# skywoodsz/qm_control

Measured on AMD Instinct MI355X. Metric: MPC+WBC control steps/sec (24-DoF quadruped-manipulator, SQP horizon N=100), higher is better.
Workload: dtype f64; 1 GPU; C3/C4: trot gait, horizon N=100 (dt 0.015), 1024 random initial states per GPU (seed 1235), cold start, 1 SQP iteration + policy eval + 3-level WBC; back-to-back steps, the WBC of a step on its own stream beside the next step's MPC kernels (pipelined THROUGHPUT: the per-kernel times add up to more than ms_per_step; the unpipelined step latency is latency_ms); instances_per_gpu=1024, global_batch=1024, parallelism=shard1, all_status_ok=True, ls_trials=1, engine=hip, max_nodes=128

## Files before the change

### qm_control_amd/csrc/host/qm_pipeline.h

```cpp
#pragma once
#include <cstddef>
#include <cstdint>
#include <vector>
#include "../kernels/k_grid.h"
#include "../kernels/k_lq.h"
#include "../kernels/k_riccati.h"
#include "../kernels/k_ls.h"
#include "../kernels/k_ilqr.h"
#include "../kernels/k_ipm.h"

struct QmMpcBuffers {
  int Bmax = 0, nmax = 0, nref = 0, nev = 0;
  double* mb = nullptr; double* st = nullptr;
  double* t0 = nullptr; double* x0 = nullptr; double* ref_t = nullptr; double* ref_x = nullptr; double* ev = nullptr; int* modes = nullptr;
  int* n_nodes = nullptr; double* node_t = nullptr; double* node_ts = nullptr; double* node_dt = nullptr; int* node_ev = nullptr; int* node_mode = nullptr;
  double* zvel = nullptr; double* zpos = nullptr; double* xref = nullptr; double* eeref = nullptr; int* status = nullptr;
  double* x = nullptr; double* u = nullptr; double* dx = nullptr; double* du = nullptr; double* stage = nullptr; double* lqdbg = nullptr; double* kin = nullptr;
  double* perf = nullptr; double* base_sum = nullptr; double* perf_sum = nullptr; double* step_info = nullptr;
  double* alpha = nullptr; int* done = nullptr; double* xs = nullptr; double* us = nullptr; double* out_perf = nullptr;
  double* xt = nullptr; double* ut = nullptr;
  double* ipm_s = nullptr; double* ipm_l = nullptr; double* ipm_ds = nullptr; double* ipm_dl = nullptr; double* ipm_ratio = nullptr; double* ipm_info = nullptr;
  int* prev_n = nullptr; double* prev_t = nullptr; int* prev_ev = nullptr;
  int* open_cnt = nullptr; int* tickets = nullptr; int* host_open_dev = nullptr; volatile int* host_open = nullptr;
  int* ncap_dev = nullptr; int* host_ncap_dev = nullptr; volatile int* host_ncap = nullptr;
};

__host__ __device__ inline int qm_mpc_status(int k0_status, const double* step_info4, bool strict) {
  if (k0_status != 0) return k0_status;
  const double* s4 = step_info4; const int pv = (s4[3] == s4[3]) ? (int)s4[3] : 2;
  const bool finite = (s4[0] - s4[0] == 0.0) && (s4[1] - s4[1] == 0.0) && (s4[2] - s4[2] == 0.0);
  if (!finite || (pv & 2)) return -4;
  if (pv & 1) return strict ? -4 : QM_MPC_WARN_PIVOT;
  return 0;
}

template <class BK>
struct QmMpcPipeline {
  BK& bk; QmMpcBuffers d;
  int ls_trials_run = 0;
  bool ls_trials_pending = false; int ls_trials_cap = 0;
  double* p0_x = nullptr; double* p0_u = nullptr; int* p0_mode = nullptr; bool p0_enable = false; bool p0_done = false;
  bool defer_apply = false; int pending_apply_B = 0; int pending_apply_threads = 0;
  bool device_tail = true;
  int riccati_skip = 0;
  int lq_prof = 0;
  int solver = 0;
  bool r_blocks = false;
  bool r_force_dense = false;
  bool rblk() const { return r_blocks && !r_force_dense; }
  bool speculative_apply = true;
  bool ipm_fresh = true;
  int solved_B = 0;
  int ncap = 0;
  bool ncap_pending = false;
  bool has_m18 = true;
  const int* front_status = nullptr; int front_B = 0;
  explicit QmMpcPipeline(BK& b) : bk(b) {}

  template <class T> T* A(size_t n) { T* p = (T*)bk.alloc(n * sizeof(T)); bk.zero(p, n * sizeof(T)); return p; }

  void allocate(const double* mb_host, const double* st_host, int Bmax, int nmax, int nref, int nev, bool debug_lq) {
    d.Bmax = Bmax; d.nmax = nmax; d.nref = nref; d.nev = nev;
    const size_t NB = (size_t)nmax * Bmax;
    d.mb = A<double>(MB_SIZE); d.st = A<double>(ST_SIZE);
    bk.to_device(d.mb, mb_host, MB_SIZE * 8); bk.to_device(d.st, st_host, ST_SIZE * 8); note_settings(st_host);
    d.t0 = A<double>(Bmax); d.x0 = A<double>((size_t)Bmax * 30); d.ref_t = A<double>((size_t)Bmax * nref); d.ref_x = A<double>((size_t)Bmax * nref * QM_NREF);
    d.ev = A<double>((size_t)Bmax * nev); d.modes = A<int>((size_t)Bmax * (nev + 1));
    d.n_nodes = A<int>(Bmax); d.node_t = A<double>(NB); d.node_ts = A<double>(NB); d.node_dt = A<double>(NB); d.node_ev = A<int>(NB); d.node_mode = A<int>(NB);
    d.zvel = A<double>(NB * 4); d.zpos = A<double>(NB * 4); d.xref = A<double>(NB * 30); d.eeref = A<double>(NB * 7); d.status = A<int>(Bmax);
    d.x = A<double>(NB * 30); d.u = A<double>(NB * 30); d.dx = A<double>(NB * 30); d.du = A<double>(NB * 30);
    d.stage = A<double>(NB * SR_SIZE); d.lqdbg = debug_lq ? A<double>(NB * LQ_DBG_SIZE) : nullptr; d.kin = A<double>((NB + 64) * KR_SIZE);
    d.perf = A<double>(NB * PF_SIZE); d.base_sum = A<double>((size_t)Bmax * 4); d.perf_sum = A<double>((size_t)Bmax * 4); d.step_info = A<double>((size_t)Bmax * 4);
    d.alpha = A<double>(Bmax); d.done = A<int>(Bmax); d.xs = A<double>(NB * 30); d.us = A<double>(NB * 30); d.out_perf = A<double>((size_t)Bmax * 10);
    d.prev_n = A<int>(Bmax); d.prev_t = A<double>(NB); d.prev_ev = A<int>(NB);
    d.open_cnt = A<int>(QM_LS_MAX_TRIALS); d.tickets = A<int>(QM_LS_MAX_TRIALS);
    d.ncap_dev = A<int>(3); { void* hv = nullptr; d.host_ncap_dev = (int*)bk.alloc_mapped(sizeof(int), &hv); d.host_ncap = (volatile int*)hv; d.host_ncap[0] = 0; }
    { void* hv = nullptr; d.host_open_dev = (int*)bk.alloc_mapped(QM_LS_MAX_TRIALS * sizeof(int), &hv); d.host_open = (volatile int*)hv; for (int i = 0; i < QM_LS_MAX_TRIALS; ++i) d.host_open[i] = 0; }
  }
  void note_settings(const double* st_host) { r_blocks = qm_r_is_block_diagonal(st_host); }
  void release() {
    void* ps[] = {d.mb, d.st, d.t0, d.x0, d.ref_t, d.ref_x, d.ev, d.modes, d.n_nodes, d.node_t, d.node_ts, d.node_dt, d.node_ev, d.node_mode, d.zvel, d.zpos, d.xref, d.eeref, d.status,
                  d.x, d.u, d.dx, d.du, d.xt, d.ut, d.ipm_s, d.ipm_l, d.ipm_ds, d.ipm_dl, d.ipm_ratio, d.ipm_info, d.stage, d.lqdbg, d.kin, d.perf, d.base_sum, d.perf_sum, d.step_info, d.alpha, d.done, d.xs, d.us, d.out_perf, d.prev_n, d.prev_t, d.prev_ev, d.open_cnt, d.tickets, d.ncap_dev};
    for (void* p : ps) if (p) bk.free(p);
    if (d.host_open) bk.free_mapped((void*)d.host_open);
    if (d.host_ncap) bk.free_mapped((void*)d.host_ncap);
    d = QmMpcBuffers();
  }

  int ls_trials() {
    if (ls_trials_pending) { int oc[QM_LS_MAX_TRIALS]; bk.to_host(oc, d.open_cnt, sizeof(oc)); int t = 0; while (t < QM_LS_MAX_TRIALS && oc[t] > 0) ++t; ls_trials_run = (1 + t > ls_trials_cap) ? ls_trials_cap : 1 + t; ls_trials_pending = false; }
    return ls_trials_run;
  }

  void apply_pending() { if (!pending_apply_B) return; QmLsArgs l = ls_args(pending_apply_B); bk.launch(qm_ls_apply_kernel, (pending_apply_threads * 30 + 255) / 256, 256, 0, l); pending_apply_B = 0; }

  void upload_inputs(int B, const double* t0, const double* x0, const double* ref_t, const double* ref_x, const double* ev, const int* modes) {
    bk.to_device(d.t0, t0, (size_t)B * 8); bk.to_device(d.x0, x0, (size_t)B * 30 * 8);
    bk.to_device(d.ref_t, ref_t, (size_t)B * d.nref * 8); bk.to_device(d.ref_x, ref_x, (size_t)B * d.nref * QM_NREF * 8);
    bk.to_device(d.ev, ev, (size_t)B * d.nev * 8); bk.to_device(d.modes, modes, (size_t)B * (d.nev + 1) * 4);
  }

  QmLsArgs ls_args(int B) {
    QmLsArgs a; a.mb = d.mb; a.st = d.st; a.B = B; a.nmax = d.nmax; a.n_nodes = d.n_nodes; a.node_ts = d.node_ts; a.node_dt = d.node_dt; a.node_ev = d.node_ev; a.node_mode = d.node_mode;
    a.zvel = d.zvel; a.zpos = d.zpos; a.xref = d.xref; a.eeref = d.eeref; a.x0 = d.x0; a.x = d.x; a.u = d.u; a.dx = d.dx; a.du = d.du; a.alpha = d.alpha; a.done = d.done;
    a.perf = d.perf; a.perf_sum = d.perf_sum; a.base_sum = d.base_sum; a.step_info = d.step_info; a.xs = d.xs; a.us = d.us; a.out_perf = d.out_perf; a.trial = 0; a.max_trials = 0; a.node_t = d.node_t; a.p0_t = d.t0; a.p0_ev = d.ev; a.p0_modes = d.modes; a.p0_nev = d.nev; a.p0_x = nullptr; a.p0_u = nullptr; a.p0_mode = nullptr; a.with_alpha = 0; a.open_cnt = d.open_cnt; a.tickets = d.tickets; a.host_open = (volatile int*)d.host_open_dev; a.xt = nullptr; a.ut = nullptr; a.ilqr = 0; a.ipm_s = nullptr; a.ipm_ds = nullptr; a.ipm_info = nullptr;
    return a;
  }

  void grid(int B, double horizon, bool warm = false) {
    warm = warm && solved_B == B;
    if (warm) { QmSaveGridArgs sg; sg.B = B; sg.nmax = d.nmax; sg.n_nodes = d.n_nodes; sg.node_t = d.node_t; sg.node_ev = d.node_ev; sg.prev_n = d.prev_n; sg.prev_t = d.prev_t; sg.prev_ev = d.prev_ev;
                bk.launch(qm_save_grid_kernel, (d.nmax * B + 63) / 64, 64, 0, sg); }
    QmGridArgs g; g.mb = d.mb; g.st = d.st; g.B = B; g.nmax = d.nmax; g.nref = d.nref; g.nev = d.nev; g.t0 = d.t0; g.x0 = d.x0; g.ref_t = d.ref_t; g.ref_x = d.ref_x; g.ev = d.ev; g.modes = d.modes;
    g.horizon = horizon; g.n_nodes = d.n_nodes; g.node_t = d.node_t; g.node_ts = d.node_ts; g.node_dt = d.node_dt; g.node_ev = d.node_ev; g.node_mode = d.node_mode;
    g.zvel = d.zvel; g.zpos = d.zpos; g.xref = d.xref; g.eeref = d.eeref; g.x = d.x; g.u = d.u; g.status = d.status; g.front_status = (front_status && front_B == B) ? front_status : nullptr;
    if (ncap_pending) bk.wait_flag(d.host_ncap, -1);
    g.ncap_dev = d.ncap_dev; g.host_ncap = (volatile int*)d.host_ncap_dev; d.host_ncap[0] = -1; ncap = 0; ncap_pending = true;
    g.warm = warm ? 1 : 0; g.prev_n = d.prev_n; g.prev_t = d.prev_t; g.prev_ev = d.prev_ev; g.prev_xs = d.xs; g.prev_us = d.us;
    bk.launch(qm_grid_kernel, (B + 63) / 64, 64, 0, g);
    bk.launch(qm_grid_nodes_kernel, (d.nmax * B + 63) / 64, 64, 0, g);
    ipm_fresh = true;
  }
  void advance(int B, double dt) {
    QmAdvanceArgs v; v.B = B; v.nmax = d.nmax; v.n_nodes = d.n_nodes; v.node_t = d.node_t; v.node_ev = d.node_ev; v.xs = d.xs; v.dt = dt; v.t0 = d.t0; v.x0 = d.x0;
    bk.launch(qm_advance_kernel, (B + 63) / 64, 64, 0, v);
  }
  void sqp_iteration(int B, int max_trials = 14, bool last = false) {
    const bool ilqr = solver == 1, ipm = solver == 3;
    QmIpmArgs ia;
    if (ipm) {
      const size_t NBm = (size_t)d.nmax * d.Bmax;
      if (!d.ipm_s) { d.ipm_s = A<double>(NBm * QM_NH); d.ipm_l = A<double>(NBm * QM_NH); d.ipm_ds = A<double>(NBm * QM_NH); d.ipm_dl = A<double>(NBm * QM_NH); d.ipm_ratio = A<double>(NBm * 2); d.ipm_info = A<double>((size_t)d.Bmax * IPM_INFO); }
      ia.mb = d.mb; ia.st = d.st; ia.B = B; ia.nmax = d.nmax; ia.n_nodes = d.n_nodes; ia.node_ev = d.node_ev; ia.node_mode = d.node_mode; ia.node_dt = d.node_dt; ia.x = d.x; ia.u = d.u; ia.dx = d.dx; ia.du = d.du;
      ia.s = d.ipm_s; ia.lam = d.ipm_l; ia.ds = d.ipm_ds; ia.dlam = d.ipm_dl; ia.ratio = d.ipm_ratio; ia.info = d.ipm_info; ia.alpha = d.alpha; ia.done = d.done; ia.out_perf = d.out_perf;
      if (ipm_fresh) bk.launch(qm_ipm_init_kernel, (d.nmax * B + 63) / 64, 64, 0, ia);
      ipm_fresh = false;
    }
    if (ilqr && !d.xt) { d.xt = A<double>((size_t)d.nmax * d.Bmax * 30); d.ut = A<double>((size_t)d.nmax * d.Bmax * 30); }
    QmRolloutArgs ro; ro.mb = d.mb; ro.st = d.st; ro.B = B; ro.nmax = d.nmax; ro.mode = 0; ro.trial = 0; ro.n_nodes = d.n_nodes; ro.node_dt = d.node_dt; ro.node_ev = d.node_ev; ro.x0 = d.x0;
    ro.x = d.x; ro.u = d.u; ro.stage = d.stage; ro.alpha = d.alpha; ro.done = d.done; ro.xt = d.xt; ro.ut = d.ut;
    if (ilqr) bk.launch(qm_ilqr_rollout_kernel, B, 64, 0, ro);
    if (ncap == 0) { if (ncap_pending) bk.wait_flag(d.host_ncap, -1); const int word = ncap_pending ? d.host_ncap[0] : (d.nmax | (1 << 16)); ncap_pending = false;
                     ncap = word & 0xFFFF; has_m18 = (word >> 16) != 0; if (ncap < 1 || ncap > d.nmax) { ncap = d.nmax; has_m18 = true; } }
    const int nodes_threads = ncap * B;
    if (max_trials > QM_LS_MAX_TRIALS) max_trials = QM_LS_MAX_TRIALS;
    QmLqArgs q; q.mb = d.mb; q.st = d.st; q.B = B; q.nmax = d.nmax; q.n_nodes = d.n_nodes; q.node_ts = d.node_ts; q.node_dt = d.node_dt; q.node_ev = d.node_ev; q.node_mode = d.node_mode;
    q.zvel = d.zvel; q.zpos = d.zpos; q.xref = d.xref; q.eeref = d.eeref; q.x = d.x; q.u = d.u; q.stage = d.stage; q.perf = d.perf; q.dbg = d.lqdbg; q.kin = d.kin; q.prof = lq_prof; q.ncap = ncap;
    q.ipm_s = d.ipm_s; q.ipm_l = d.ipm_l; q.ipm_info = d.ipm_info; q.rb = rblk() ? 1 : 0; q.single_mt = has_m18 ? 0 : 1;
    q.i0 = 0;
    bk.launch(qm_lq_kin_kernel, (nodes_threads + 63) / 64, 64, LQ_KIN_LDS_BYTES, q);
    if (ipm) bk.launch(qm_lq_ipm_kernel, B * ncap, LW_BLOCK, LQ_LDS_BYTES, q);
    else if (d.lqdbg || lq_prof) bk.launch(qm_lq_dbg_kernel, B * ncap, LW_BLOCK, LQ_LDS_BYTES, q);
    else { bk.launch(qm_lq_kernel, B * ncap, LW_BLOCK, LQ_LDS_BYTES, q);
           if (has_m18) bk.launch(qm_lq_m18_kernel, B * ncap, LW_BLOCK, LQ_LDS_BYTES, q); }
    QmLsArgs l = ls_args(B); if (ilqr) { l.xt = d.xt; l.ut = d.ut; l.ilqr = 1; }
    if (ipm) { l.ipm_s = d.ipm_s; l.ipm_ds = d.ipm_ds; l.ipm_info = d.ipm_info; }
    QmRiccatiArgs r; r.B = B; r.nmax = d.nmax; r.n_nodes = d.n_nodes; r.node_ev = d.node_ev; r.x0 = d.x0; r.x = d.x; r.stage = d.stage; r.dx = d.dx; r.du = d.du; r.step_info = d.step_info; r.skip = riccati_skip;
    r.perf = d.perf; r.base_sum = d.base_sum; r.alpha = d.alpha; r.done = d.done; r.out_perf = d.out_perf; r.open_cnt = d.open_cnt; r.tickets = d.tickets;
    if (riccati_skip) bk.launch(qm_riccati_prof_kernel, B, RW_BLOCK, RW_LDS_BYTES, r);
    else bk.launch(qm_riccati_kernel, B, RW_BLOCK, RW_LDS_BYTES, r);
    if (ipm) { bk.launch(qm_ipm_dir_kernel, (d.nmax * B + 63) / 64, 64, 0, ia); bk.launch(qm_ipm_alpha_kernel, B, 64, 0, ia); }
    ls_trials_run = 0; ls_trials_pending = false; p0_done = false;
    if (device_tail && !ilqr && !ipm && max_trials >= 1) {
      l.trial = 0; l.max_trials = max_trials;
      if (p0_enable && last && p0_x) { l.p0_x = p0_x; l.p0_u = p0_u; l.p0_mode = p0_mode; p0_done = true; bk.wbc_inputs_next(); }
      if (rblk()) bk.launch(qm_ls_eval_kernel, (nodes_threads + 63) / 64, 64, LS_EVAL_LDS_BYTES, l); else bk.launch(qm_ls_eval_dense_kernel, (nodes_threads + 63) / 64, 64, LS_EVAL_LDS_BYTES, l);
      { QmLsArgs ls = l; ls.with_alpha = 1; ls.tickets = nullptr; bk.launch(qm_perf_sum_kernel, B, 64, 0, ls); }
      if (max_trials > 1) { QmLsArgs lt = l; lt.trial = 1;
        if (rblk()) bk.launch(qm_ls_tail_kernel, B, LS_TAIL_BLOCK, LS_TAIL_LDS_BYTES(d.nmax), lt); else bk.launch(qm_ls_tail_dense_kernel, B, LS_TAIL_BLOCK, LS_TAIL_LDS_BYTES(d.nmax), lt); }
      ls_trials_pending = true; ls_trials_cap = max_trials;
      if (defer_apply && last) { pending_apply_B = B; pending_apply_threads = nodes_threads; solved_B = B; return; }
      bk.launch(qm_ls_apply_kernel, (nodes_threads * 30 + 255) / 256, 256, 0, l);
      if (!last) bk.launch(qm_ls_commit_kernel, (nodes_threads * 30 + 255) / 256, 256, 0, l);
// ... 23 lines not shown
```

### qm_control_amd/csrc/host/qmhip.hip

```cpp
#include <hip/hip_runtime.h>
#include <chrono>
#include <cmath>
#include <cstdio>
#include <cstring>
#include <map>
#include <mutex>
#include <string>
#include <vector>
#include "../../../include/qmhip.h"
#include "qm_model_io.h"
#define QM_LQ_KERNELS_EXTERN 1
#include "qm_pipeline.h"
#include "qm_wbc_pipeline.h"
#include "qm_sim_pipeline.h"
#include "qm_front_pipeline.h"
#include "qm_hoqp_pipeline.h"
#include "qm_io_pipeline.h"
#include "qm_tick_pipeline.h"
#include "qm_publish_pipeline.h"

static thread_local std::string g_create_error;

#define QM_GUARD(c) std::unique_lock<std::recursive_mutex> qm_lk_; if (c) qm_lk_ = std::unique_lock<std::recursive_mutex>(const_cast<qmhip_ctx*>(c)->mu)
#define QM_NEED_MPC(c) do { if ((c) && (c)->wbc_only) { const_cast<qmhip_ctx*>(c)->fail(std::string(__func__) + ": not available on a WBC-only context (qmhip_create_wbc_context)"); return QMHIP_ERR_STATE; } } while (0)
#define HIP_TRY(ctx, expr) do { hipError_t e_ = (expr); if (e_ != hipSuccess) { (ctx)->fail(std::string(#expr) + ": " + hipGetErrorString(e_)); return QMHIP_ERR_HIP; } } while (0)

struct HipBackend {
  hipStream_t stream = nullptr;
  hipStream_t stream_b = nullptr;
  hipStream_t stream_c = nullptr;
  hipStream_t cur = nullptr;
  hipEvent_t ev_in = nullptr, ev_wbc = nullptr; bool wbc_pending = false;
  int profiling = 0;
  std::string error;
  struct Span { std::string name; hipEvent_t a, b; };
  std::vector<Span> spans; std::vector<hipEvent_t> pool;
  std::map<std::string, std::pair<double, int>> acc;
  std::map<const void*, int> lds_set;
  std::map<std::string, int> lds_pad;
  hipEvent_t ev() { if (!pool.empty()) { hipEvent_t e = pool.back(); pool.pop_back(); return e; } hipEvent_t e = nullptr; check(hipEventCreate(&e), "hipEventCreate"); return e; }
  void check(hipError_t e, const char* what) { if (e != hipSuccess && error.empty()) error = std::string(what) + ": " + hipGetErrorString(e); }
  template <class K> const char* name_of(K k) {
    const void* p = (const void*)k;
    if (p == (const void*)qm_grid_kernel || p == (const void*)qm_grid_nodes_kernel || p == (const void*)qm_save_grid_kernel || p == (const void*)qm_advance_kernel) return "grid"; if (p == (const void*)qm_lq_kernel || p == (const void*)qm_lq_dbg_kernel || p == (const void*)qm_lq_ipm_kernel) return "lq"; if (p == (const void*)qm_lq_m18_kernel) return "lq_m18"; if (p == (const void*)qm_lq_kin_kernel) return "lq_kin"; if (p == (const void*)qm_riccati_kernel || p == (const void*)qm_riccati_prof_kernel) return "riccati";
    if (p == (const void*)qm_ls_eval_kernel || p == (const void*)qm_ls_eval_dense_kernel || p == (const void*)qm_ls_eval_ipm_kernel) return "ls_eval";
    if (p == (const void*)qm_ipm_init_kernel || p == (const void*)qm_ipm_dir_kernel || p == (const void*)qm_ipm_alpha_kernel || p == (const void*)qm_ipm_commit_kernel || p == (const void*)qm_ipm_barrier_kernel) return "ipm"; if (p == (const void*)qm_ilqr_rollout_kernel) return "rollout"; if (p == (const void*)qm_sim_kernel) return "sim"; if (p == (const void*)qm_wbc_kernel || p == (const void*)qm_wbc_prof_kernel) return "wbc"; if (p == (const void*)qm_policy_kernel || p == (const void*)qm_policy_measured_kernel) return "policy"; if (p == (const void*)qm_policy_fb_kernel || p == (const void*)qm_policy_fb_pub_kernel) return "policy_fb"; if (p == (const void*)qm_policy_publish_kernel) return "publish"; if (p == (const void*)qm_hoqp_kernel) return "hoqp"; if (p == (const void*)qm_step_pack_kernel) return "io"; if (p == (const void*)qm_tick_state_kernel || p == (const void*)qm_tick_pack_kernel) return "tick";
    return "ls_misc";
  }
  template <class K, class A> void launch(K kernel, int grid, int block, size_t lds, const A& args) {
    if (grid <= 0) return;
    if (!lds_pad.empty()) { auto it = lds_pad.find(name_of(kernel)); if (it != lds_pad.end()) lds += (size_t)it->second; }
    if (lds > 48 * 1024) {
      const void* p = (const void*)kernel; auto it = lds_set.find(p);
      if (it == lds_set.end() || it->second < (int)lds) { check(hipFuncSetAttribute(p, hipFuncAttributeMaxDynamicSharedMemorySize, (int)lds), "hipFuncSetAttribute"); lds_set[p] = (int)lds; }
    }
    const void* kp_ = (const void*)kernel;
    const bool is_lq_ = kp_ == (const void*)qm_lq_kernel || kp_ == (const void*)qm_lq_m18_kernel || kp_ == (const void*)qm_lq_ipm_kernel;
    const bool span = profiling == 1 || (profiling == 3 && is_lq_) || (profiling == 2 && (kp_ == (const void*)qm_lq_kernel || kp_ == (const void*)qm_lq_m18_kernel || kp_ == (const void*)qm_lq_ipm_kernel || kp_ == (const void*)qm_riccati_kernel || kp_ == (const void*)qm_wbc_kernel));
    Span s; if (span) { s.name = name_of(kernel); s.a = ev(); s.b = ev(); check(hipEventRecord(s.a, cur), "hipEventRecord"); }
    hipLaunchKernelGGL(kernel, dim3(grid), dim3(block), lds, cur, args);
    check(hipGetLastError(), "kernel launch");
    if (span) { check(hipEventRecord(s.b, cur), "hipEventRecord"); spans.push_back(s); }
  }
  void resolve() {
    if (spans.empty()) return;
    hipStreamSynchronize(stream); hipStreamSynchronize(stream_b);
    for (auto& s : spans) { float ms = 0; hipEventElapsedTime(&ms, s.a, s.b); auto& a = acc[s.name]; a.first += ms; a.second += 1; pool.push_back(s.a); pool.push_back(s.b); }
    spans.clear();
  }
  void* alloc(size_t n) { void* p = nullptr; check(hipMalloc(&p, n ? n : 8), "hipMalloc"); return p; }
  void free(void* p) { hipFree(p); }
  void zero(void* p, size_t n) { check(hipMemsetAsync(p, 0, n, cur), "hipMemsetAsync"); }
  void to_device(void* d, const void* s, size_t n) { sync(); check(hipMemcpyAsync(d, s, n, hipMemcpyHostToDevice, stream), "H2D"); check(hipStreamSynchronize(stream), "sync"); }
  void to_host(void* d, const void* s, size_t n) { sync(); check(hipMemcpyAsync(d, s, n, hipMemcpyDeviceToHost, stream), "D2H"); check(hipStreamSynchronize(stream), "sync"); }
  void sync() { check(hipStreamSynchronize(stream), "sync"); check(hipStreamSynchronize(stream_b), "sync"); wbc_pending = false; }
  hipEvent_t ev_order = nullptr;
  void stream_select(int s) { cur = s ? stream_b : stream; }
  void stream_order(int a, int b) { if (!ev_order) check(hipEventCreateWithFlags(&ev_order, hipEventDisableTiming), "hipEventCreate"); check(hipEventRecord(ev_order, a ? stream_b : stream), "hipEventRecord"); check(hipStreamWaitEvent(b ? stream_b : stream, ev_order, 0), "hipStreamWaitEvent"); }
  void copy_dd(void* d, const void* s, size_t n) { check(hipMemcpyAsync(d, s, n, hipMemcpyDeviceToDevice, cur), "D2D"); }
  void* alloc_mapped(size_t n, void** host_view) { void* h = nullptr; void* dv = nullptr; check(hipHostMalloc(&h, n ? n : 8, hipHostMallocMapped), "hipHostMalloc"); check(hipHostGetDevicePointer(&dv, h, 0), "hipHostGetDevicePointer"); *host_view = h; return dv; }
  void free_mapped(void* host_view) { hipHostFree(host_view); }
  hipEvent_t ev_io_a = nullptr, ev_io_b = nullptr;
  void* alloc_pinned(size_t n) { void* h = nullptr; check(hipHostMalloc(&h, n ? n : 8, hipHostMallocDefault), "hipHostMalloc"); return h; }
  void free_pinned(void* p) { hipHostFree(p); }
  void* io_event() { hipEvent_t e = nullptr; check(hipEventCreateWithFlags(&e, hipEventDisableTiming), "hipEventCreate"); return (void*)e; }
  void io_event_free(void* e) { hipEventDestroy((hipEvent_t)e); }
  void copy_in(void* d, const void* s, size_t n, int on) { check(hipMemcpyAsync(d, s, n, hipMemcpyHostToDevice, on ? stream_b : stream), "H2D"); }
  void copy_out(void* d, const void* s, size_t n, void* done, bool wbc) {
    if (!ev_io_a) { check(hipEventCreateWithFlags(&ev_io_a, hipEventDisableTiming), "hipEventCreate"); check(hipEventCreateWithFlags(&ev_io_b, hipEventDisableTiming), "hipEventCreate"); }
    check(hipEventRecord(ev_io_a, stream), "hipEventRecord"); check(hipStreamWaitEvent(stream_c, ev_io_a, 0), "hipStreamWaitEvent");
    if (wbc) { check(hipEventRecord(ev_io_b, stream_b), "hipEventRecord"); check(hipStreamWaitEvent(stream_c, ev_io_b, 0), "hipStreamWaitEvent"); }
    check(hipMemcpyAsync(d, s, n, hipMemcpyDeviceToHost, stream_c), "D2H"); check(hipEventRecord((hipEvent_t)done, stream_c), "hipEventRecord");
  }
  void copy_back(void* d, const void* s, size_t n, void* done) { check(hipMemcpyAsync(d, s, n, hipMemcpyDeviceToHost, stream), "D2H"); check(hipEventRecord((hipEvent_t)done, stream), "hipEventRecord"); }
  void* pub_event() { return io_event(); }
  void pub_event_free(void* e) { io_event_free(e); }
  void pub_wait(void* e) { check(hipStreamWaitEvent(cur, (hipEvent_t)e, 0), "hipStreamWaitEvent"); }
// ... 630 lines not shown
```

### qm_control_amd/csrc/kernels/k_grid.h

```cpp
#pragma once
#include "qm_dev_common.h"

#define QM_WEAK_EPS 1e-6
#define QM_LIMIT_EPS 2.220446049250313e-16

struct QmGridArgs {
  const double* mb; const double* st;
  int B, nmax, nref, nev;
  const double* t0;
  const double* x0;
  const double* ref_t;
  const double* ref_x;
  const double* ev;
  const int* modes;
  double horizon;
  int* n_nodes;
  double* node_t;
  double* node_ts;
  double* node_dt;
  int* node_ev;
  int* node_mode;
  double* zvel; double* zpos;
  double* xref;
  double* eeref;
  int* ncap_dev; volatile int* host_ncap;
  double* x; double* u;
  int warm; const int* prev_n; const double* prev_t; const int* prev_ev; const double* prev_xs; const double* prev_us;
  int* status;
  const int* front_status;
};

__device__ __forceinline__ int grid_find_index(const double* ev, int nev, double t) {
  int k = 0; while (k < nev && ev[k] < t) ++k; return k;
}
__device__ __forceinline__ void cubic_eval(double t0, double p0, double v0, double t1, double p1, double v1, double t, double* pos, double* vel) {
  const double dt = t1 - t0, dp = p1 - p0, dv = v1 - v0;
  const double c0 = p0, c1 = v0 * dt, c2 = -(3.0 * v0 + dv) * dt + 3.0 * dp, c3 = (2.0 * v0 + dv) * dt - 2.0 * dp;
  const double s = (t - t0) / dt;
  *pos = c3 * s * s * s + c2 * s * s + c1 * s + c0;
  *vel = (3.0 * c3 * s * s + 2.0 * c2 * s + c1) / dt;
}
__device__ __forceinline__ void grid_time_segment(const double* ta, int n, double t, int* index, double* alpha) {
  if (n <= 1) { *index = 0; *alpha = 1.0; return; }
  const int part = grid_find_index(ta, n, t);
  const int interval = (part == 0 && t == ta[0]) ? 0 : part - 1;
  const int last = n - 1;
  if (interval >= 0) {
    if (interval < last) {
      const double len = ta[interval + 1] - ta[interval], till = ta[interval + 1] - t;
      *index = interval;
      *alpha = (len > 2.0 * QM_WEAK_EPS) ? till / len : ((till > 0.5 * len) ? 1.0 : 0.0);
    } else { *index = (last - 1 > 0) ? last - 1 : 0; *alpha = 0.0; }
  } else { *index = 0; *alpha = 1.0; }
}

__global__ void qm_grid_kernel(QmGridArgs a) {
  const int b = blockIdx.x * blockDim.x + threadIdx.x;
  int n = 0, has18 = 0;
  if (b < a.B) {
  const double* ev = a.ev + (size_t)b * a.nev; const int* modes = a.modes + (size_t)b * (a.nev + 1);
  const double t0 = a.t0[b], tf = t0 + a.horizon, dt = qm_ms_param(a.st, ST_SQP_DT);
  const double dtMin = a.st[ST_GRID_DT_MIN];
  int status = a.front_status ? a.front_status[b] : 0;
  a.node_t[0 * a.B + b] = t0; a.node_ev[0 * a.B + b] = QM_EV_NONE; n = 1;
  int k = grid_find_index(ev, a.nev, t0);
  double nt = t0; double backT = t0;
  const bool sane = dt > 0.0 && dt < 1.0e300 && t0 == t0 && tf > t0 && tf < 1.0e300;
  if (!sane) status = (status == 0) ? -1 : status;
  while (sane && backT < tf) {
    nt = nt + dt; int nevt = QM_EV_NONE; bool post = false;
    if (k < a.nev && nt >= ev[k]) { nt = ev[k]; nevt = QM_EV_PRE; post = true; ++k; }
    if (nt >= tf) { nt = tf; nevt = QM_EV_NONE; post = false; }
    if (nt > backT + dtMin) { if (n >= a.nmax) { status = (status == 0) ? -1 : status; break; } a.node_t[n * a.B + b] = nt; a.node_ev[n * a.B + b] = nevt; ++n; }
    else { a.node_t[(n - 1) * a.B + b] = nt; a.node_ev[(n - 1) * a.B + b] = nevt; }
    backT = nt;
    if (post) { if (n >= a.nmax) { status = (status == 0) ? -1 : status; break; } a.node_t[n * a.B + b] = nt; a.node_ev[n * a.B + b] = QM_EV_POST; ++n; }
  }
  a.n_nodes[b] = n;
  a.status[b] = status;
  { const int k0 = grid_find_index(ev, a.nev, t0), k1e = grid_find_index(ev, a.nev, tf + QM_WEAK_EPS), k1 = (k1e < a.nev) ? k1e : a.nev;
    for (int q = k0; q <= k1; ++q) { const int mq = modes[q]; if ((int)mode_flag(mq, 0) + (int)mode_flag(mq, 1) + (int)mode_flag(mq, 2) + (int)mode_flag(mq, 3) >= 3) has18 = 1; } }
  }
  if (a.ncap_dev) {
    double m = (double)n, h = (double)has18;
    for (int off = 32; off > 0; off >>= 1) { m = fmax(m, __shfl_xor(m, off, 64)); h = fmax(h, __shfl_xor(h, off, 64)); }
    if ((threadIdx.x & 63) == 0) {
      atomicMax(a.ncap_dev, (int)m); if (h > 0.0) atomicOr(a.ncap_dev + 2, 1); __threadfence();
      if (atomicAdd(a.ncap_dev + 1, 1) == (int)gridDim.x - 1) { const int f18 = atomicOr(a.ncap_dev + 2, 0); a.host_ncap[0] = atomicMax(a.ncap_dev, 0) | (f18 << 16); a.ncap_dev[0] = 0; a.ncap_dev[1] = 0; a.ncap_dev[2] = 0; __threadfence_system(); }
    }
  }
}

__device__ __forceinline__ void grid_policy_segment(const double* node_t, const int* node_ev, int n, int B, int b, double t, int* index, double* alpha) {
  auto tt = [&](int i) { const int e = node_ev[i * B + b]; return node_t[i * B + b] + (e == QM_EV_POST ? QM_LIMIT_EPS : (e == QM_EV_PRE ? -QM_LIMIT_EPS : 0.0)); };
  int part = 0; while (part < n && tt(part) < t) ++part;
  const int interval = (part == 0 && t == tt(0)) ? 0 : part - 1; const int last = n - 1;
  if (n <= 1) { *index = 0; *alpha = 1.0; }
  else if (interval >= 0) {
    if (interval < last) { const double len = tt(interval + 1) - tt(interval), till = tt(interval + 1) - t; *index = interval; *alpha = (len > 2.0 * QM_WEAK_EPS) ? till / len : ((till > 0.5 * len) ? 1.0 : 0.0); }
    else { *index = (last - 1 > 0) ? last - 1 : 0; *alpha = 0.0; }
  } else { *index = 0; *alpha = 1.0; }
}

__global__ void QM_MAX_VGPRS(72) qm_grid_nodes_kernel(QmGridArgs a) {
  const int g = blockIdx.x * blockDim.x + threadIdx.x;
  const int i = g / a.B, b = g - i * a.B;
  if (i >= a.nmax) return;
  const int n = a.n_nodes[b];
  if (i >= n) return;
  const double* ev = a.ev + (size_t)b * a.nev; const int* modes = a.modes + (size_t)b * (a.nev + 1);
  int status = 0;
  const double mass = a.mb[MB_ROBOTMASS];
  const double liftV = a.st[ST_LIFTOFF_VEL], touchV = a.st[ST_TOUCHDOWN_VEL], swingH = a.st[ST_SWING_HEIGHT], tScale = a.st[ST_SWING_TIME_SCALE];
  const double* rt = a.ref_t + (size_t)b * a.nref; const double* rx = a.ref_x + (size_t)b * a.nref * QM_NREF;
  {
    const int nb = i * a.B + b;
    const double t = a.node_t[nb]; const int e = a.node_ev[nb];
    const double ts = (e == QM_EV_POST) ? t + QM_WEAK_EPS : t;
    double d = 0.0;
    if (i < n - 1 && e != QM_EV_PRE) { const double tn = a.node_t[(i + 1) * a.B + b]; const int en = a.node_ev[(i + 1) * a.B + b]; d = ((en == QM_EV_PRE) ? tn - QM_WEAK_EPS : tn) - ts; }
    a.node_ts[nb] = ts; a.node_dt[nb] = d;
    const int p = grid_find_index(ev, a.nev, ts); const int mode = modes[p];
    a.node_mode[nb] = mode;
    for (int c = 0; c < 4; ++c) {
      double zp = 0.0, zv = 0.0;
      if (!mode_flag(mode, c)) {
        int s = -1; for (int ip = p - 1; ip >= 0; --ip) if (mode_flag(modes[ip], c)) { s = ip; break; }
        int f = -1; for (int ip = p + 1; ip <= a.nev; ++ip) if (mode_flag(modes[ip], c)) { f = ip - 1; break; }
        if (s < 0 || f < 0) { status = (status == 0) ? -2 : status; }
        else {
          const double tsw = ev[s], tew = ev[f]; const double sc = fmin(1.0, (tew - tsw) / tScale); const double mid = (tsw + tew) / 2.0;
          if (ts < mid) cubic_eval(tsw, 0.0, sc * liftV, mid, sc * swingH, 0.0, ts, &zp, &zv);
          else cubic_eval(mid, sc * swingH, 0.0, tew, 0.0, sc * touchV, ts, &zp, &zv);
        }
      }
      a.zvel[nb * 4 + c] = zv; a.zpos[nb * 4 + c] = zp;
    }
    {
      int idx; double al; grid_time_segment(rt, a.nref, ts, &idx, &al);
      if (a.nref == 1) { for (int q = 0; q < 30; ++q) a.xref[nb * 30 + q] = rx[q]; for (int q = 0; q < 7; ++q) a.eeref[nb * 7 + q] = rx[30 + q]; }
      else {
        const double* l = rx + idx * QM_NREF; const double* r = rx + (idx + 1) * QM_NREF;
        for (int q = 0; q < 30; ++q) a.xref[nb * 30 + q] = al * l[q] + (1.0 - al) * r[q];
        for (int q = 0; q < 3; ++q) a.eeref[nb * 7 + q] = al * l[30 + q] + (1.0 - al) * r[30 + q];
        const double* ql = l + 33; const double* qr = r + 33; const double tt = 1.0 - al; const double one = 1.0 - QM_LIMIT_EPS;
        const double dd = ql[0] * qr[0] + ql[1] * qr[1] + ql[2] * qr[2] + ql[3] * qr[3]; const double ad = fabs(dd); double s0, s1;
        if (ad >= one) { s0 = 1.0 - tt; s1 = tt; } else { const double th = acos(ad), sth = sin(th); s0 = sin((1.0 - tt) * th) / sth; s1 = sin(tt * th) / sth; }
        if (dd < 0.0) s1 = -s1;
        for (int q = 0; q < 4; ++q) a.eeref[nb * 7 + 3 + q] = s0 * ql[q] + s1 * qr[q];
      }
    }
    int nst = 0; for (int c = 0; c < 4; ++c) nst += mode_flag(mode, c);
    const int np = (a.warm && a.prev_n) ? a.prev_n[b] : 0;
    const double tend = (np >= 2) ? a.prev_t[(np - 1) * a.B + b] : 0.0;
    auto istart = [&](int j) { const double tj = a.node_t[j * a.B + b]; return (a.node_ev[j * a.B + b] == QM_EV_POST) ? tj + QM_WEAK_EPS : tj; };
    auto iend = [&](int j) { const double tj = a.node_t[j * a.B + b]; return (a.node_ev[j * a.B + b] == QM_EV_PRE) ? tj - QM_WEAK_EPS : tj; };
    auto covered = [&](int j) { return np >= 2 && j < n - 1 && a.node_ev[j * a.B + b] != QM_EV_PRE && !(istart(j) > tend || iend(j + 1) > tend); };
    int j = i; while (j > 0 && !covered(j - 1)) --j;
    if (j == 0) { for (int q = 0; q < 30; ++q) a.x[nb * 30 + q] = a.x0[(size_t)b * 30 + q]; }
    else {
      int idx; double al; grid_policy_segment(a.prev_t, a.prev_ev, np, a.B, b, iend(j), &idx, &al);
      const double* x0p = a.prev_xs + (size_t)(idx * a.B + b) * 30; const double* x1p = a.prev_xs + (size_t)((idx + 1) * a.B + b) * 30;
      for (int q = 0; q < 30; ++q) a.x[nb * 30 + q] = al * x0p[q] + (1.0 - al) * x1p[q];
    }
    if (covered(i)) {
      int idx; double al; grid_policy_segment(a.prev_t, a.prev_ev, np, a.B, b, ts, &idx, &al);
      const double* u0p = a.prev_us + (size_t)(idx * a.B + b) * 30; const double* u1p = a.prev_us + (size_t)((idx + 1) * a.B + b) * 30;
      for (int q = 0; q < 30; ++q) a.u[nb * 30 + q] = al * u0p[q] + (1.0 - al) * u1p[q];
    } else {
      for (int q = 0; q < 30; ++q) a.u[nb * 30 + q] = 0.0;
      if (e != QM_EV_PRE && nst > 0) for (int c = 0; c < 4; ++c) if (mode_flag(mode, c)) a.u[nb * 30 + 3 * c + 2] = mass * 9.81 / nst;
    }
  }
  if (status != 0 && a.status[b] == 0) a.status[b] = status;
}

struct QmSaveGridArgs { int B, nmax; const int* n_nodes; const double* node_t; const int* node_ev; int* prev_n; double* prev_t; int* prev_ev; };
__global__ void qm_save_grid_kernel(QmSaveGridArgs a) {
  const int g = blockIdx.x * blockDim.x + threadIdx.x;
  const int i = g / a.B, b = g - i * a.B;
  if (i >= a.nmax) return;
  if (i == 0) a.prev_n[b] = a.n_nodes[b];
  if (i < a.n_nodes[b]) { a.prev_t[g] = a.node_t[g]; a.prev_ev[g] = a.node_ev[g]; }
}
struct QmAdvanceArgs { int B, nmax; const int* n_nodes; const double* node_t; const int* node_ev; const double* xs; double dt; double* t0; double* x0; };
__global__ void qm_advance_kernel(QmAdvanceArgs a) {
  const int b = blockIdx.x * blockDim.x + threadIdx.x;
  if (b >= a.B) return;
  const double t = a.t0[b] + a.dt;
  int idx; double al; grid_policy_segment(a.node_t, a.node_ev, a.n_nodes[b], a.B, b, t, &idx, &al);
  const int i1 = (a.n_nodes[b] > 1) ? idx + 1 : idx;
  for (int q = 0; q < 30; ++q) a.x0[(size_t)b * 30 + q] = al * a.xs[(size_t)(idx * a.B + b) * 30 + q] + (1.0 - al) * a.xs[(size_t)(i1 * a.B + b) * 30 + q];
  a.t0[b] = t;
}
```

Measured before the change: 440,000 steps/s.

## Parallelize grid construction: wavefront-per-instance event search and per-row fill kernel

```diff
diff --git a/qm_control_amd/csrc/host/qm_pipeline.h b/qm_control_amd/csrc/host/qm_pipeline.h
--- a/qm_control_amd/csrc/host/qm_pipeline.h
+++ b/qm_control_amd/csrc/host/qm_pipeline.h
@@ -23,6 +23,7 @@
   int* prev_n = nullptr; double* prev_t = nullptr; int* prev_ev = nullptr;
   int* open_cnt = nullptr; int* tickets = nullptr; int* host_open_dev = nullptr; volatile int* host_open = nullptr;
   int* ncap_dev = nullptr; int* host_ncap_dev = nullptr; volatile int* host_ncap = nullptr;
+  double* dsc_d = nullptr; int* dsc_i = nullptr;
 };
 
 __host__ __device__ inline int qm_mpc_status(int k0_status, const double* step_info4, bool strict) {
@@ -72,7 +73,7 @@
     d.stage = A<double>(NB * SR_SIZE); d.lqdbg = debug_lq ? A<double>(NB * LQ_DBG_SIZE) : nullptr; d.kin = A<double>((NB + 64) * KR_SIZE);
     d.perf = A<double>(NB * PF_SIZE); d.base_sum = A<double>((size_t)Bmax * 4); d.perf_sum = A<double>((size_t)Bmax * 4); d.step_info = A<double>((size_t)Bmax * 4);
     d.alpha = A<double>(Bmax); d.done = A<int>(Bmax); d.xs = A<double>(NB * 30); d.us = A<double>(NB * 30); d.out_perf = A<double>((size_t)Bmax * 10);
-    d.prev_n = A<int>(Bmax); d.prev_t = A<double>(NB); d.prev_ev = A<int>(NB);
+    d.prev_n = A<int>(Bmax); d.prev_t = A<double>(NB); d.prev_ev = A<int>(NB); d.dsc_d = A<double>(NB * GD_N); d.dsc_i = A<int>(NB * GI_N);
     d.open_cnt = A<int>(QM_LS_MAX_TRIALS); d.tickets = A<int>(QM_LS_MAX_TRIALS);
     d.ncap_dev = A<int>(3); { void* hv = nullptr; d.host_ncap_dev = (int*)bk.alloc_mapped(sizeof(int), &hv); d.host_ncap = (volatile int*)hv; d.host_ncap[0] = 0; }
     { void* hv = nullptr; d.host_open_dev = (int*)bk.alloc_mapped(QM_LS_MAX_TRIALS * sizeof(int), &hv); d.host_open = (volatile int*)hv; for (int i = 0; i < QM_LS_MAX_TRIALS; ++i) d.host_open[i] = 0; }
@@ -80,7 +81,7 @@
   void note_settings(const double* st_host) { r_blocks = qm_r_is_block_diagonal(st_host); }
   void release() {
     void* ps[] = {d.mb, d.st, d.t0, d.x0, d.ref_t, d.ref_x, d.ev, d.modes, d.n_nodes, d.node_t, d.node_ts, d.node_dt, d.node_ev, d.node_mode, d.zvel, d.zpos, d.xref, d.eeref, d.status,
-                  d.x, d.u, d.dx, d.du, d.xt, d.ut, d.ipm_s, d.ipm_l, d.ipm_ds, d.ipm_dl, d.ipm_ratio, d.ipm_info, d.stage, d.lqdbg, d.kin, d.perf, d.base_sum, d.perf_sum, d.step_info, d.alpha, d.done, d.xs, d.us, d.out_perf, d.prev_n, d.prev_t, d.prev_ev, d.open_cnt, d.tickets, d.ncap_dev};
+                  d.x, d.u, d.dx, d.du, d.xt, d.ut, d.ipm_s, d.ipm_l, d.ipm_ds, d.ipm_dl, d.ipm_ratio, d.ipm_info, d.stage, d.lqdbg, d.kin, d.perf, d.base_sum, d.perf_sum, d.step_info, d.alpha, d.done, d.xs, d.us, d.out_perf, d.prev_n, d.prev_t, d.prev_ev, d.open_cnt, d.tickets, d.ncap_dev, d.dsc_d, d.dsc_i};
     for (void* p : ps) if (p) bk.free(p);
     if (d.host_open) bk.free_mapped((void*)d.host_open);
     if (d.host_ncap) bk.free_mapped((void*)d.host_ncap);
@@ -113,12 +114,13 @@
                 bk.launch(qm_save_grid_kernel, (d.nmax * B + 63) / 64, 64, 0, sg); }
     QmGridArgs g; g.mb = d.mb; g.st = d.st; g.B = B; g.nmax = d.nmax; g.nref = d.nref; g.nev = d.nev; g.t0 = d.t0; g.x0 = d.x0; g.ref_t = d.ref_t; g.ref_x = d.ref_x; g.ev = d.ev; g.modes = d.modes;
     g.horizon = horizon; g.n_nodes = d.n_nodes; g.node_t = d.node_t; g.node_ts = d.node_ts; g.node_dt = d.node_dt; g.node_ev = d.node_ev; g.node_mode = d.node_mode;
-    g.zvel = d.zvel; g.zpos = d.zpos; g.xref = d.xref; g.eeref = d.eeref; g.x = d.x; g.u = d.u; g.status = d.status; g.front_status = (front_status && front_B == B) ? front_status : nullptr;
+    g.zvel = d.zvel; g.zpos = d.zpos; g.xref = d.xref; g.eeref = d.eeref; g.x = d.x; g.u = d.u; g.dsc_d = d.dsc_d; g.dsc_i = d.dsc_i; g.status = d.status; g.front_status = (front_status && front_B == B) ? front_status : nullptr;
     if (ncap_pending) bk.wait_flag(d.host_ncap, -1);
     g.ncap_dev = d.ncap_dev; g.host_ncap = (volatile int*)d.host_ncap_dev; d.host_ncap[0] = -1; ncap = 0; ncap_pending = true;
     g.warm = warm ? 1 : 0; g.prev_n = d.prev_n; g.prev_t = d.prev_t; g.prev_ev = d.prev_ev; g.prev_xs = d.xs; g.prev_us = d.us;
-    bk.launch(qm_grid_kernel, (B + 63) / 64, 64, 0, g);
+    bk.launch(qm_grid_kernel, B, 64, 0, g);
     bk.launch(qm_grid_nodes_kernel, (d.nmax * B + 63) / 64, 64, 0, g);
+    bk.launch(qm_grid_rows_kernel, (int)(((size_t)d.nmax * B * 30 + 255) / 256), 256, 0, g);
     ipm_fresh = true;
   }
   void advance(int B, double dt) {
diff --git a/qm_control_amd/csrc/host/qmhip.hip b/qm_control_amd/csrc/host/qmhip.hip
--- a/qm_control_amd/csrc/host/qmhip.hip
+++ b/qm_control_amd/csrc/host/qmhip.hip
@@ -42,7 +42,7 @@
   void check(hipError_t e, const char* what) { if (e != hipSuccess && error.empty()) error = std::string(what) + ": " + hipGetErrorString(e); }
   template <class K> const char* name_of(K k) {
     const void* p = (const void*)k;
-    if (p == (const void*)qm_grid_kernel || p == (const void*)qm_grid_nodes_kernel || p == (const void*)qm_save_grid_kernel || p == (const void*)qm_advance_kernel) return "grid"; if (p == (const void*)qm_lq_kernel || p == (const void*)qm_lq_dbg_kernel || p == (const void*)qm_lq_ipm_kernel) return "lq"; if (p == (const void*)qm_lq_m18_kernel) return "lq_m18"; if (p == (const void*)qm_lq_kin_kernel) return "lq_kin"; if (p == (const void*)qm_riccati_kernel || p == (const void*)qm_riccati_prof_kernel) return "riccati";
+    if (p == (const void*)qm_grid_kernel || p == (const void*)qm_grid_nodes_kernel || p == (const void*)qm_grid_rows_kernel || p == (const void*)qm_save_grid_kernel || p == (const void*)qm_advance_kernel) return "grid"; if (p == (const void*)qm_lq_kernel || p == (const void*)qm_lq_dbg_kernel || p == (const void*)qm_lq_ipm_kernel) return "lq"; if (p == (const void*)qm_lq_m18_kernel) return "lq_m18"; if (p == (const void*)qm_lq_kin_kernel) return "lq_kin"; if (p == (const void*)qm_riccati_kernel || p == (const void*)qm_riccati_prof_kernel) return "riccati";
     if (p == (const void*)qm_ls_eval_kernel || p == (const void*)qm_ls_eval_dense_kernel || p == (const void*)qm_ls_eval_ipm_kernel) return "ls_eval";
     if (p == (const void*)qm_ipm_init_kernel || p == (const void*)qm_ipm_dir_kernel || p == (const void*)qm_ipm_alpha_kernel || p == (const void*)qm_ipm_commit_kernel || p == (const void*)qm_ipm_barrier_kernel) return "ipm"; if (p == (const void*)qm_ilqr_rollout_kernel) return "rollout"; if (p == (const void*)qm_sim_kernel) return "sim"; if (p == (const void*)qm_wbc_kernel || p == (const void*)qm_wbc_prof_kernel) return "wbc"; if (p == (const void*)qm_policy_kernel || p == (const void*)qm_policy_measured_kernel) return "policy"; if (p == (const void*)qm_policy_fb_kernel || p == (const void*)qm_policy_fb_pub_kernel) return "policy_fb"; if (p == (const void*)qm_policy_publish_kernel) return "publish"; if (p == (const void*)qm_hoqp_kernel) return "hoqp"; if (p == (const void*)qm_step_pack_kernel) return "io"; if (p == (const void*)qm_tick_state_kernel || p == (const void*)qm_tick_pack_kernel) return "tick";
     return "ls_misc";
diff --git a/qm_control_amd/csrc/kernels/k_grid.h b/qm_control_amd/csrc/kernels/k_grid.h
--- a/qm_control_amd/csrc/kernels/k_grid.h
+++ b/qm_control_amd/csrc/kernels/k_grid.h
@@ -25,10 +25,22 @@
   double* eeref;
   int* ncap_dev; volatile int* host_ncap;
   double* x; double* u;
+  double* dsc_d; int* dsc_i;
   int warm; const int* prev_n; const double* prev_t; const int* prev_ev; const double* prev_xs; const double* prev_us;
   int* status;
   const int* front_status;
 };
+
+#define GD_AL 0
+#define GD_S0 1
+#define GD_S1 2
+#define GD_XAL 3
+#define GD_UAL 4
+#define GD_N 5
+#define GI_REF 0
+#define GI_X 1
+#define GI_U 2
+#define GI_N 3
 
 __device__ __forceinline__ int grid_find_index(const double* ev, int nev, double t) {
   int k = 0; while (k < nev && ev[k] < t) ++k; return k;
@@ -54,40 +66,51 @@
   } else { *index = 0; *alpha = 1.0; }
 }
 
-__global__ void qm_grid_kernel(QmGridArgs a) {
-  const int b = blockIdx.x * blockDim.x + threadIdx.x;
+__global__ void QM_MAX_VGPRS(72) qm_grid_kernel(QmGridArgs a) {
+  const int b = blockIdx.x, l = threadIdx.x & 63;
   int n = 0, has18 = 0;
   if (b < a.B) {
   const double* ev = a.ev + (size_t)b * a.nev; const int* modes = a.modes + (size_t)b * (a.nev + 1);
+  const double w0 = (l < a.nev) ? ev[l] : 0.0;
   const double t0 = a.t0[b], tf = t0 + a.horizon, dt = qm_ms_param(a.st, ST_SQP_DT);
   const double dtMin = a.st[ST_GRID_DT_MIN];
   int status = a.front_status ? a.front_status[b] : 0;
-  a.node_t[0 * a.B + b] = t0; a.node_ev[0 * a.B + b] = QM_EV_NONE; n = 1;
-  int k = grid_find_index(ev, a.nev, t0);
+  auto find = [&](double t) -> int {
+    for (int c = 0; c < a.nev; c += 64) {
+      const double v = (c == 0) ? w0 : ((c + l < a.nev) ? ev[c + l] : 0.0);
+      const unsigned long long m = __ballot(c + l >= a.nev || !(v < t));
+      if (m) return c + __ffsll((long long)m) - 1;
+    }
+    return a.nev;
+  };
+  int wbase = 0; double win = w0;
+  auto ev_at = [&](int k) -> double {
+    if (k - wbase >= 64) { wbase = k; win = (k + l < a.nev) ? ev[k + l] : 0.0; }
+    return qm_bcast(win, k - wbase);
+  };
+  const int k0 = find(t0);
+  { const int k1e = find(tf + QM_WEAK_EPS), k1 = (k1e < a.nev) ? k1e : a.nev; int f = 0;
+    for (int c = k0; c <= k1; c += 64) if (c + l <= k1) { const int mq = modes[c + l]; if ((int)mode_flag(mq, 0) + (int)mode_flag(mq, 1) + (int)mode_flag(mq, 2) + (int)mode_flag(mq, 3) >= 3) f = 1; }
+    has18 = __ballot(f) != 0ull; }
+  if (l == 0) { a.node_t[0 * a.B + b] = t0; a.node_ev[0 * a.B + b] = QM_EV_NONE; } n = 1;
+  int k = k0; double evk = (k < a.nev) ? ev_at(k) : 0.0;
   double nt = t0; double backT = t0;
   const bool sane = dt > 0.0 && dt < 1.0e300 && t0 == t0 && tf > t0 && tf < 1.0e300;
   if (!sane) status = (status == 0) ? -1 : status;
   while (sane && backT < tf) {
     nt = nt + dt; int nevt = QM_EV_NONE; bool post = false;
-    if (k < a.nev && nt >= ev[k]) { nt = ev[k]; nevt = QM_EV_PRE; post = true; ++k; }
+    if (k < a.nev && nt >= evk) { nt = evk; nevt = QM_EV_PRE; post = true; ++k; evk = (k < a.nev) ? ev_at(k) : 0.0; }
     if (nt >= tf) { nt = tf; nevt = QM_EV_NONE; post = false; }
-    if (nt > backT + dtMin) { if (n >= a.nmax) { status = (status == 0) ? -1 : status; break; } a.node_t[n * a.B + b] = nt; a.node_ev[n * a.B + b] = nevt; ++n; }
-    else { a.node_t[(n - 1) * a.B + b] = nt; a.node_ev[(n - 1) * a.B + b] = nevt; }
+    if (nt > backT + dtMin) { if (n >= a.nmax) { status = (status == 0) ? -1 : status; break; } if (l == 0) { a.node_t[n * a.B + b] = nt; a.node_ev[n * a.B + b] = nevt; } ++n; }
+    else if (l == 0) { a.node_t[(n - 1) * a.B + b] = nt; a.node_ev[(n - 1) * a.B + b] = nevt; }
     backT = nt;
-    if (post) { if (n >= a.nmax) { status = (status == 0) ? -1 : status; break; } a.node_t[n * a.B + b] = nt; a.node_ev[n * a.B + b] = QM_EV_POST; ++n; }
-  }
-  a.n_nodes[b] = n;
-  a.status[b] = status;
-  { const int k0 = grid_find_index(ev, a.nev, t0), k1e = grid_find_index(ev, a.nev, tf + QM_WEAK_EPS), k1 = (k1e < a.nev) ? k1e : a.nev;
-    for (int q = k0; q <= k1; ++q) { const int mq = modes[q]; if ((int)mode_flag(mq, 0) + (int)mode_flag(mq, 1) + (int)mode_flag(mq, 2) + (int)mode_flag(mq, 3) >= 3) has18 = 1; } }
-  }
-  if (a.ncap_dev) {
-    double m = (double)n, h = (double)has18;
-    for (int off = 32; off > 0; off >>= 1) { m = fmax(m, __shfl_xor(m, off, 64)); h = fmax(h, __shfl_xor(h, off, 64)); }
-    if ((threadIdx.x & 63) == 0) {
-      atomicMax(a.ncap_dev, (int)m); if (h > 0.0) atomicOr(a.ncap_dev + 2, 1); __threadfence();
-      if (atomicAdd(a.ncap_dev + 1, 1) == (int)gridDim.x - 1) { const int f18 = atomicOr(a.ncap_dev + 2, 0); a.host_ncap[0] = atomicMax(a.ncap_dev, 0) | (f18 << 16); a.ncap_dev[0] = 0; a.ncap_dev[1] = 0; a.ncap_dev[2] = 0; __threadfence_system(); }
-    }
+    if (post) { if (n >= a.nmax) { status = (status == 0) ? -1 : status; break; } if (l == 0) { a.node_t[n * a.B + b] = nt; a.node_ev[n * a.B + b] = QM_EV_POST; } ++n; }
+  }
+  if (l == 0) { a.n_nodes[b] = n; a.status[b] = status; }
+  }
+  if (a.ncap_dev && l == 0) {
+    atomicMax(a.ncap_dev, n); if (has18) atomicOr(a.ncap_dev + 2, 1); __threadfence();
+    if (atomicAdd(a.ncap_dev + 1, 1) == (int)gridDim.x - 1) { const int f18 = atomicOr(a.ncap_dev + 2, 0); a.host_ncap[0] = atomicMax(a.ncap_dev, 0) | (f18 << 16); a.ncap_dev[0] = 0; a.ncap_dev[1] = 0; a.ncap_dev[2] = 0; __threadfence_system(); }
   }
 }
 
@@ -110,9 +133,9 @@
   if (i >= n) return;
   const double* ev = a.ev + (size_t)b * a.nev; const int* modes = a.modes + (size_t)b * (a.nev + 1);
   int status = 0;
-  const double mass = a.mb[MB_ROBOTMASS];
   const double liftV = a.st[ST_LIFTOFF_VEL], touchV = a.st[ST_TOUCHDOWN_VEL], swingH = a.st[ST_SWING_HEIGHT], tScale = a.st[ST_SWING_TIME_SCALE];
   const double* rt = a.ref_t + (size_t)b * a.nref; const double* rx = a.ref_x + (size_t)b * a.nref * QM_NREF;
+  const size_t P = (size_t)a.nmax * a.B;
   {
     const int nb = i * a.B + b;
     const double t = a.node_t[nb]; const int e = a.node_ev[nb];
@@ -136,43 +159,64 @@
       }
       a.zvel[nb * 4 + c] = zv; a.zpos[nb * 4 + c] = zp;
     }
-    {
+    if (a.nref != 1) {
       int idx; double al; grid_time_segment(rt, a.nref, ts, &idx, &al);
-      if (a.nref == 1) { for (int q = 0; q < 30; ++q) a.xref[nb * 30 + q] = rx[q]; for (int q = 0; q < 7; ++q) a.eeref[nb * 7 + q] = rx[30 + q]; }
-      else {
-        const double* l = rx + idx * QM_NREF; const double* r = rx + (idx + 1) * QM_NREF;
-        for (int q = 0; q < 30; ++q) a.xref[nb * 30 + q] = al * l[q] + (1.0 - al) * r[q];
-        for (int q = 0; q < 3; ++q) a.eeref[nb * 7 + q] = al * l[30 + q] + (1.0 - al) * r[30 + q];
-        const double* ql = l + 33; const double* qr = r + 33; const double tt = 1.0 - al; const double one = 1.0 - QM_LIMIT_EPS;
-        const double dd = ql[0] * qr[0] + ql[1] * qr[1] + ql[2] * qr[2] + ql[3] * qr[3]; const double ad = fabs(dd); double s0, s1;
-        if (ad >= one) { s0 = 1.0 - tt; s1 = tt; } else { const double th = acos(ad), sth = sin(th); s0 = sin((1.0 - tt) * th) / sth; s1 = sin(tt * th) / sth; }
-        if (dd < 0.0) s1 = -s1;
-        for (int q = 0; q < 4; ++q) a.eeref[nb * 7 + 3 + q] = s0 * ql[q] + s1 * qr[q];
-      }
+      a.dsc_i[GI_REF * P + nb] = idx; a.dsc_d[GD_AL * P + nb] = al;
+      const double* l = rx + idx * QM_NREF; const double* r = rx + (idx + 1) * QM_NREF;
+      const double* ql = l + 33; const double* qr = r + 33; const double tt = 1.0 - al; const double one = 1.0 - QM_LIMIT_EPS;
+      const double dd = ql[0] * qr[0] + ql[1] * qr[1] + ql[2] * qr[2] + ql[3] * qr[3]; const double ad = fabs(dd); double s0, s1;
+      if (ad >= one) { s0 = 1.0 - tt; s1 = tt; } else { const double th = acos(ad), sth = sin(th); s0 = sin((1.0 - tt) * th) / sth; s1 = sin(tt * th) / sth; }
+      if (dd < 0.0) s1 = -s1;
+      a.dsc_d[GD_S0 * P + nb] = s0; a.dsc_d[GD_S1 * P + nb] = s1;
     }
-    int nst = 0; for (int c = 0; c < 4; ++c) nst += mode_flag(mode, c);
     const int np = (a.warm && a.prev_n) ? a.prev_n[b] : 0;
     const double tend = (np >= 2) ? a.prev_t[(np - 1) * a.B + b] : 0.0;
     auto istart = [&](int j) { const double tj = a.node_t[j * a.B + b]; return (a.node_ev[j * a.B + b] == QM_EV_POST) ? tj + QM_WEAK_EPS : tj; };
     auto iend = [&](int j) { const double tj = a.node_t[j * a.B + b]; return (a.node_ev[j * a.B + b] == QM_EV_PRE) ? tj - QM_WEAK_EPS : tj; };
     auto covered = [&](int j) { return np >= 2 && j < n - 1 && a.node_ev[j * a.B + b] != QM_EV_PRE && !(istart(j) > tend || iend(j + 1) > tend); };
     int j = i; while (j > 0 && !covered(j - 1)) --j;
-    if (j == 0) { for (int q = 0; q < 30; ++q) a.x[nb * 30 + q] = a.x0[(size_t)b * 30 + q]; }
-    else {
-      int idx; double al; grid_policy_segment(a.prev_t, a.prev_ev, np, a.B, b, iend(j), &idx, &al);
-      const double* x0p = a.prev_xs + (size_t)(idx * a.B + b) * 30; const double* x1p = a.prev_xs + (size_t)((idx + 1) * a.B + b) * 30;
-      for (int q = 0; q < 30; ++q) a.x[nb * 30 + q] = al * x0p[q] + (1.0 - al) * x1p[q];
-    }
-    if (covered(i)) {
-      int idx; double al; grid_policy_segment(a.prev_t, a.prev_ev, np, a.B, b, ts, &idx, &al);
-      const double* u0p = a.prev_us + (size_t)(idx * a.B + b) * 30; const double* u1p = a.prev_us + (size_t)((idx + 1) * a.B + b) * 30;
-      for (int q = 0; q < 30; ++q) a.u[nb * 30 + q] = al * u0p[q] + (1.0 - al) * u1p[q];
-    } else {
-      for (int q = 0; q < 30; ++q) a.u[nb * 30 + q] = 0.0;
-      if (e != QM_EV_PRE && nst > 0) for (int c = 0; c < 4; ++c) if (mode_flag(mode, c)) a.u[nb * 30 + 3 * c + 2] = mass * 9.81 / nst;
-    }
+    if (j == 0) a.dsc_i[GI_X * P + nb] = -1;
+    else { int idx; double al; grid_policy_segment(a.prev_t, a.prev_ev, np, a.B, b, iend(j), &idx, &al); a.dsc_i[GI_X * P + nb] = idx; a.dsc_d[GD_XAL * P + nb] = al; }
+    if (covered(i)) { int idx; double al; grid_policy_segment(a.prev_t, a.prev_ev, np, a.B, b, ts, &idx, &al); a.dsc_i[GI_U * P + nb] = idx; a.dsc_d[GD_UAL * P + nb] = al; }
+    else a.dsc_i[GI_U * P + nb] = -1;
   }
   if (status != 0 && a.status[b] == 0) a.status[b] = status;
+}
+
+__global__ void QM_MAX_VGPRS(72) qm_grid_rows_kernel(QmGridArgs a) {
+  const size_t P = (size_t)a.nmax * a.B;
+  const size_t g = (size_t)blockIdx.x * blockDim.x + threadIdx.x;
+  if (g >= P * 30) return;
+  const int nb = (int)(g / 30), q = (int)(g - (size_t)nb * 30);
+  const int i = nb / a.B, b = nb - i * a.B;
+  if (i >= a.n_nodes[b]) return;
+  const double* rx = a.ref_x + (size_t)b * a.nref * QM_NREF;
+  if (a.nref == 1) { a.xref[g] = rx[q]; if (q < 7) a.eeref[(size_t)nb * 7 + q] = rx[30 + q]; }
+  else {
+    const int idx = a.dsc_i[GI_REF * P + nb]; const double al = a.dsc_d[GD_AL * P + nb];
+    const double* l = rx + idx * QM_NREF; const double* r = rx + (idx + 1) * QM_NREF;
+    a.xref[g] = al * l[q] + (1.0 - al) * r[q];
+    if (q < 3) a.eeref[(size_t)nb * 7 + q] = al * l[30 + q] + (1.0 - al) * r[30 + q];
+    else if (q < 7) { const double s0 = a.dsc_d[GD_S0 * P + nb], s1 = a.dsc_d[GD_S1 * P + nb]; const double* ql = l + 33; const double* qr = r + 33; a.eeref[(size_t)nb * 7 + q] = s0 * ql[q - 3] + s1 * qr[q - 3]; }
+  }
+  const int xi = a.dsc_i[GI_X * P + nb];
+  if (xi < 0) a.x[g] = a.x0[(size_t)b * 30 + q];
+  else {
+    const double al = a.dsc_d[GD_XAL * P + nb];
+    const double* x0p = a.prev_xs + (size_t)(xi * a.B + b) * 30; const double* x1p = a.prev_xs + (size_t)((xi + 1) * a.B + b) * 30;
+    a.x[g] = al * x0p[q] + (1.0 - al) * x1p[q];
+  }
+  const int ui = a.dsc_i[GI_U * P + nb];
+  if (ui >= 0) {
+    const double al = a.dsc_d[GD_UAL * P + nb];
+    const double* u0p = a.prev_us + (size_t)(ui * a.B + b) * 30; const double* u1p = a.prev_us + (size_t)((ui + 1) * a.B + b) * 30;
+    a.u[g] = al * u0p[q] + (1.0 - al) * u1p[q];
+  } else {
+    const int mode = a.node_mode[nb]; int nst = 0; for (int c = 0; c < 4; ++c) nst += mode_flag(mode, c);
+    const int c = q / 3; const double mass = a.mb[MB_ROBOTMASS];
+    const bool fz = q < 12 && q - 3 * c == 2 && a.node_ev[nb] != QM_EV_PRE && nst > 0 && mode_flag(mode, c);
+    a.u[g] = fz ? mass * 9.81 / nst : 0.0;
+  }
 }
 
 struct QmSaveGridArgs { int B, nmax; const int* n_nodes; const double* node_t; const int* node_ev; int* prev_n; double* prev_t; int* prev_ev; };
```

Measured after the change: 434,400 steps/s. 1.3% lower.
